# dcmlr/groundgrid

Hardware: NVIDIA H100
Metric: Mpoints/sec segmented (64-beam scan) (higher is better)
Workload: dtype f32/f64

## Files before the change

### groundgrid_b200/csrc/gg_capi.cu

```cuda
#include <cuda.h>
#include <cuda_runtime.h>

#include <cmath>
#include <cstdarg>
#include <cstdio>
#include <algorithm>
#include <atomic>
#include <chrono>
#include <condition_variable>
#include <cstdlib>
#include <cstring>
#include <initializer_list>
#include <mutex>
#include <string>
#include <thread>
#include <utility>
#include <vector>

#include "gg_host.h"
#include "gg_internal.h"

namespace {

thread_local std::string g_last_error;
// ... 1077 lines not shown
    h->have_layer_map = encode_layer_map(h);
    float* expected = nullptr;
    GG_TRY(dev_alloc(h, &expected, N2));
    v.expected = expected;
    GG_TRY(dev_alloc(h, &v.points, S * P));
    GG_TRY(dev_alloc(h, &v.zw, S * P));
    GG_TRY(dev_alloc(h, &v.zsorted, S * P));
    GG_TRY(dev_alloc(h, &v.runj, S * P));
    GG_TRY(dev_alloc(h, &v.rundir, S * P));
    GG_TRY(dev_alloc(h, &v.dist, S * P));
    GG_TRY(dev_alloc(h, &v.code, S * P));
    GG_TRY(dev_alloc(h, &v.labels, S * P));
    GG_TRY(dev_alloc(h, &v.cnt64, S * N2));
    GG_TRY(dev_alloc(h, &v.raw_i, (flags & GG_FLAG_FULL_LAYERS) ? S * N2 : 1));
    GG_TRY(dev_alloc(h, &v.cellstart, S * N2));
    GG_TRY(dev_alloc(h, &v.worklist, S * N2));
    GG_TRY(dev_alloc(h, &v.wl_count, 2 * S));
    v.cell_tiles = (int)((N2 + 4095) / 4096);
    GG_TRY(dev_alloc(h, &v.cell_agg, S * v.cell_tiles * 65));
    GG_TRY(dev_alloc(h, &v.out_index, S * P));
    GG_TRY(dev_alloc(h, &v.out_counts, S * (3 * (size_t)v.out_blocks + 1)));
    GG_TRY(dev_alloc(h, &v.roll_scratch, S * 2 * N2));
    v.out_cloud = nullptr;
    GG_CUDA_TRY(cudaMemset(v.layers, 0, S * v.n_layers * N2 * sizeof(float)));
    GG_CUDA_TRY(cudaMemset(v.cnt64, 0, S * N2 * sizeof(unsigned long long)));
    if (flags & GG_FLAG_FULL_LAYERS) GG_CUDA_TRY(cudaMemset(v.raw_i, 0, S * N2 * sizeof(int)));

    {
        std::vector<float> table;
        gg::build_expected_points(n, table);
        GG_CUDA_TRY(cudaMemcpy(expected, table.data(), N2 * sizeof(float), cudaMemcpyHostToDevice));
        gg::SpiralPlan plan;
        gg::plan_spiral(n, v.k.res_sq, plan);
        GG_TRY(dev_upload(h, &v.level_start, plan.level_start));
        GG_TRY(dev_upload(h, &v.visits, plan.visits, 1));
        v.levels = (int)plan.level_start.size() - 1;
        h->sched_levels = v.levels;
        h->sched_visits = (int)plan.visits.size();
        h->sched_max = plan.max_per_level;
        v.spiral_threads = plan.threads;
        v.spiral_recs = nullptr;
        std::memset(&v.skew, 0, sizeof(v.skew));
        if (plan.kind == gg::SPIRAL_PIPE) {
            const uint32_t* d_rc = nullptr;
            GG_TRY(dev_upload(h, &d_rc, plan.recs, 4));
            v.spiral_recs = reinterpret_cast<const uint4*>(d_rc);
        } else if (plan.kind == gg::SPIRAL_SKEW) {
            const gg::SkewTables& sk = plan.skew;
            gg::SkewView& w = v.skew;
            GG_TRY(dev_upload(h, &w.ph_begin, plan.ph_begin));
            GG_TRY(dev_upload(h, &w.ph_end, plan.ph_end));
            GG_TRY(dev_upload(h, &w.ph_cell0, plan.ph_cell0));
            GG_TRY(dev_upload(h, &w.cell_home, sk.cell_home));
            const uint32_t* d_irr = nullptr;
            GG_TRY(dev_upload(h, &d_irr, plan.irr_blocks, 16));
            float2* d_sk = nullptr;
            float* d_sd = nullptr;
            GG_TRY(dev_alloc(h, &d_sk, S * sk.slots));
            GG_TRY(dev_alloc(h, &d_sd, S * sk.slots));
            GG_CUDA_TRY(cudaMemset(d_sk, 0, S * sk.slots * sizeof(float2)));
            GG_CUDA_TRY(cudaMemset(d_sd, 0, S * sk.slots * sizeof(float)));
            w.sk = d_sk;
            w.sd = d_sd;
            w.slots = sk.slots;
            w.M = plan.M;
            w.phases = plan.phases;
            w.irr_blocks = reinterpret_cast<const uint4*>(d_irr);
            w.irr_max = plan.irr_max;
            w.irr_chunks = plan.irr_chunks;
            w.KP = sk.KP;
            w.rows = sk.rows;
            w.row0 = sk.row0;
            w.lanes = sk.lanes;
            w.levels = sk.levels;
            std::memcpy(w.pattern, sk.pattern, sizeof(sk.pattern));
        }
    }

    if (const char* e = getenv("GG_LAUNCH_UNIT")) h->launch_unit = std::max(1, atoi(e));
    if (const char* e = getenv("GG_HOST_PACK")) {
        h->host_pack = atoi(e) ? 1 : 0;
        h->host_pack_mix = 0;
    }
    v.packed = nullptr;
    if (stream) {
        h->own_streams = false;
        h->n_streams = 1;
        h->streams[0] = static_cast<cudaStream_t>(stream);
    } else {
        int want = 8;
        if (const char* e = getenv("GG_STREAMS")) want = atoi(e);
        h->n_streams = std::max(1, std::min(std::min(want, kStreams), n_slots));
        for (int i = 0; i < h->n_streams; ++i) GG_CUDA_TRY(cudaStreamCreateWithFlags(&h->streams[i], cudaStreamNonBlocking));
    }
    GG_CUDA_TRY(cudaHostAlloc(reinterpret_cast<void**>(&h->h_ring), sizeof(gg::SlotParams) * kRing * S, cudaHostAllocDefault));
    GG_TRY(dev_alloc(h, &h->d_ring, (size_t)kRing * S));
    GG_CUDA_TRY(cudaHostAlloc(reinterpret_cast<void**>(&h->h_dest), sizeof(gg::OutDest) * kRing * S, cudaHostAllocDefault));
    GG_TRY(dev_alloc(h, &h->d_dest, (size_t)kRing * S));
    GG_CUDA_TRY(cudaHostAlloc(reinterpret_cast<void**>(&h->h_unpack), sizeof(gg::UnpackDesc) * kRing * S, cudaHostAllocDefault));
    GG_TRY(dev_alloc(h, &h->d_unpack, (size_t)kRing * S));
    GG_CUDA_TRY(cudaHostAlloc(reinterpret_cast<void**>(&h->h_query), sizeof(gg::QueryDesc) * kRing * S, cudaHostAllocDefault));
    GG_TRY(dev_alloc(h, &h->d_query, (size_t)kRing * S));
    for (int i = 0; i < kRing; ++i) GG_CUDA_TRY(cudaEventCreateWithFlags(&h->ring_ev[i], cudaEventDisableTiming));
    GG_CUDA_TRY(cudaEventCreateWithFlags(&h->caller_in, cudaEventDisableTiming));
    for (int i = 0; i < kStreams; ++i) GG_CUDA_TRY(cudaEventCreateWithFlags(&h->caller_out[i], cudaEventDisableTiming));
    GG_TRY(build_variant(h, 0, h->streams[0]));
// ... 1791 lines not shown
```

### groundgrid_b200/csrc/gg_host.cpp

```cpp
#include <immintrin.h>

#include <algorithm>
#include <cmath>
#include <cstdio>
#include <thread>
#include <cstdint>
#include <cstdlib>
#include <cstring>
#include <vector>

#include <sched.h>

#include "gg_host.h"

namespace gg {

int cells_per_side(double dimension_m, float resolution) {
    return (int)std::round((float)dimension_m / resolution);
}

void build_expected_points(int n, std::vector<float>& table) {
    const float vertical_point_ang_dist = 0.00174532925 * 2;
    table.assign((size_t)n * n, 0.0f);
    const size_t cells = (size_t)n;
// ... 186 lines not shown
    std::vector<Visit> seq;
    seq.reserve(nv);
    std::vector<int> seen((size_t)n * n, 0);
    int max_level = 0;
    auto push = [&](int s, int k, int j, int x, int y) {
        const size_t cell = x + (size_t)y * n;
        const int l = cell_levels[cell][seen[cell]++];
        seq.push_back({s, k, j, x, y, l});
        max_level = std::max(max_level, l);
    };
    for (int k = 0; k < K; ++k) {
        const int p = c - 1 - k, L = 2 * (k + 1), q = p + L;
        for (int j = 0; j < L; ++j) push(0, k, j, p, p + j);
        for (int j = 0; j < L; ++j) push(1, k, j, p + j, p);
        for (int j = 0; j <= L; ++j) push(2, k, j, q, q - j);
        for (int j = 0; j <= L; ++j) push(3, k, j, q - j, q);
    }
    if (seq.size() != nv) return;
    int off[4] = {0, 0, 0, 0};
    const int k_ref = K / 2;
    for (const Visit& v : seq)
        if (v.k == k_ref && v.j == 0) off[v.s] = v.level - 3 * k_ref;
    for (const Visit& v : seq)
        if (v.k >= 4 && v.j == 0 && v.level != 3 * v.k + off[v.s]) return;
    const int LK = 2 * (K + 1);
    t.rows = std::max(max_level, 3 * K + off[3] + LK + 1) + t.row0 + 8;
    t.lanes = 4 * t.KP;
    t.slots = (size_t)4 * t.rows * t.KP;
    auto slot = [&](int s, int k, int level) { return (int)(((size_t)s * t.rows + level + t.row0) * t.KP + (k + 1)); };

    t.cell_home.assign((size_t)n * n * 4, -1);
    auto add_home = [&](int x, int y, int sl) {
        int* h = &t.cell_home[((size_t)x + (size_t)y * n) * 4];
        for (int i = 0; i < 4; ++i)
            if (h[i] < 0) {
                h[i] = sl;
                return;
            }
    };
    for (const Visit& v : seq) add_home(v.x, v.y, slot(v.s, v.k, v.level));
    {
        const int p = 0, k = K, q = p + LK;
        if (q < n) {
            for (int j = 0; j < LK; ++j) add_home(p, p + j, slot(0, k, 3 * k + off[0] + j));
            for (int j = 1; j < LK; ++j) add_home(p + j, p, slot(1, k, 3 * k + off[1] + j));
            for (int j = 0; j <= LK; ++j) add_home(q, q - j, slot(2, k, 3 * k + off[2] + j));
            for (int j = 1; j <= LK; ++j)
                if (!(q - j == p)) add_home(q - j, q, slot(3, k, 3 * k + off[3] + j));
            add_home(p, q, slot(3, k, 3 * k + off[3] + LK));
        }
        for (int s = 0; s < 4; ++s) add_home(c, c, slot(s, -1, -3 + off[s]));
    }
    auto homes = [&](int x, int y) { return &t.cell_home[((size_t)x + (size_t)y * n) * 4]; };

    std::vector<std::vector<std::pair<int, int>>> stat(36);
    auto bump = [&](int idx, int o) {
        for (auto& e : stat[idx])
            if (e.first == o) {
                ++e.second;
                return;
            }
        stat[idx].push_back({o, 1});
    };
    for (const Visit& v : seq) {
        if (v.j < 3 || v.k < 4) continue;
        const int own = slot(v.s, v.k, v.level);
        for (int q = 0; q < 9; ++q) {
            const int* h = homes(v.x - 1 + q % 3, v.y - 1 + q / 3);
            for (int i = 0; i < 4 && h[i] >= 0; ++i) bump(v.s * 9 + q, h[i] - own);
        }
    }
    for (int i = 0; i < 36; ++i) {
        int best = 0, cnt = -1;
        for (auto& e : stat[i])
            if (e.second > cnt) {
                cnt = e.second;
                best = e.first;
            }
        if (cnt < 0) return;
        t.pattern[i] = best;
    }

    std::vector<int> last_level((size_t)n * n, -1000000), last_lane((size_t)n * n, -1);
    t.lane_begin.assign(t.lanes, 0);
    t.lane_end.assign(t.lanes, 0);
    t.lane_cell0.assign(t.lanes, 0);
    std::vector<int> reg_first(t.lanes, -1), reg_last(t.lanes, -1), reg_count(t.lanes, 0);
    struct Irr {
        int level;
        uint32_t w[16];
    };
    std::vector<Irr> irr;
    for (const Visit& v : seq) {
        const int lane = v.s * t.KP + (v.k + 1);
        const int own = slot(v.s, v.k, v.level);
        const size_t cell = v.x + (size_t)v.y * n;
        int nb[9];
        bool regular = true;
        uint32_t rec[4] = {0xffffu, 0xffffu, 0xffffu, 0xffffu};
        int nrec = 0;
        for (int q = 0; q < 9; ++q) {
            const int cx = v.x - 1 + q % 3, cy = v.y - 1 + q / 3;
            const int* h = homes(cx, cy);
            if (h[0] < 0) return;
            const int want = own + t.pattern[v.s * 9 + q];
            bool match = false;
// ... 272 lines not shown
    std::memcpy(dst, t.data(), t.size() * sizeof(float));
    return n;
}

int gg_host_spiral_schedule(int n, int* level_start, int level_cap, uint32_t* visits, int visit_cap, int* n_levels, int* n_visits) {
    std::vector<int> ls;
    std::vector<uint32_t> vs;
    gg::build_spiral_schedule(n, ls, vs);
    *n_levels = (int)ls.size() - 1;
    *n_visits = (int)vs.size();
    if (level_start && level_cap >= (int)ls.size()) std::memcpy(level_start, ls.data(), ls.size() * sizeof(int));
    if (visits && visit_cap >= (int)vs.size()) std::memcpy(visits, vs.data(), vs.size() * sizeof(uint32_t));
    return 0;
}

int gg_host_spiral_records(int n, float resolution, int dist, uint32_t* recs, int rec_cap_words, int* max_recent) {
    std::vector<int> ls;
    std::vector<uint32_t> vs, rc;
    gg::build_spiral_schedule(n, ls, vs);
    int mr = 0;
    const bool ok = gg::build_spiral_records(n, (double)resolution * (double)resolution, ls, vs, dist, rc, mr);
    if (max_recent) *max_recent = mr;
    if (recs && rec_cap_words >= (int)rc.size()) std::memcpy(recs, rc.data(), rc.size() * sizeof(uint32_t));
    return ok ? 1 : 0;
}

int gg_host_spiral_plan(int n, float resolution, int* out) {
    gg::SpiralPlan p;
    gg::plan_spiral(n, (double)resolution * (double)resolution, p);
    const int v[4] = {(int)p.kind, p.threads, p.M, p.phases};
    std::memcpy(out, v, sizeof(v));
    return 0;
}

int gg_host_spiral_skew(int n, int* header, int* pattern, int* lane_begin, int* lane_end, int* cell_home, int* irr_level_start,
                        uint32_t* irr_recs, int irr_cap_words) {
    std::vector<int> ls;
    std::vector<uint32_t> vs;
    gg::build_spiral_schedule(n, ls, vs);
    gg::SkewTables t;
    gg::build_spiral_skew(n, ls, vs, t);
    const int h[10] = {t.ok ? 1 : 0, t.K, t.KP, t.rows, t.levels, t.row0, t.lanes, (int)t.n_irregular, t.max_irr_per_level, (int)t.n_regular};
    std::memcpy(header, h, sizeof(h));
    if (!t.ok) return 0;
    if (pattern) std::memcpy(pattern, t.pattern, sizeof(t.pattern));
    if (lane_begin) std::memcpy(lane_begin, t.lane_begin.data(), t.lane_begin.size() * sizeof(int));
    if (lane_end) std::memcpy(lane_end, t.lane_end.data(), t.lane_end.size() * sizeof(int));
    if (cell_home) std::memcpy(cell_home, t.cell_home.data(), t.cell_home.size() * sizeof(int));
    if (irr_level_start) std::memcpy(irr_level_start, t.irr_level_start.data(), t.irr_level_start.size() * sizeof(int));
    if (irr_recs && irr_cap_words >= (int)t.irr_recs.size()) std::memcpy(irr_recs, t.irr_recs.data(), t.irr_recs.size() * sizeof(uint32_t));
    return 1;
}

int gg_host_decay_confidence(const gg_config* cfg, const float* occ, size_t n, float* out) {
    gg::CfgConst k;
    gg::derive_config(*cfg, k);
    for (size_t i = 0; i < n; ++i) out[i] = gg::decay_confidence(k, occ[i]);
    return 0;
}

int gg_host_skew_visit_confidence(const float* d, const float* occ, size_t n, float* out) {
    for (size_t i = 0; i < n; ++i) out[i] = gg::skew_decays(d[i]) ? d[i] : occ[i];
    return 0;
}

int gg_host_outlier_walk(double dimension_m, float resolution, const double* pos_xy, const float* G, const float* C, double thr, double tol,
                         const float* origin, const float* point, long long from) {
    gg::Const k;
    gg::derive_geometry(dimension_m, resolution, 0, k);
    float vx = point[0] - origin[0], vy = point[1] - origin[1], vz = point[2] - origin[2];
    const float sq = (vx * vx + vy * vy) + vz * vz;
    const float len = std::sqrt(sq);
    vx = vx / len;
    vy = vy / len;
    vz = vz / len;
    if (!(vz < -0.01f)) return -1;
    if (from < 0) return -1;
    const gg::OutlierRay ray{pos_xy[0], pos_xy[1], k.half, k.res, (double)len * (double)len, thr, tol, origin[0], origin[1], origin[2], vx, vy, vz, k.N};
    return gg::outlier_walk(ray, G, C, from > 2147483648LL ? 2147483648u : (unsigned)from) ? 1 : 0;
}

int gg_host_move_map(double res, double* pos_xy, double nx, double ny, int* shift_ij) {
    gg::move_map(res, pos_xy[0], pos_xy[1], nx, ny, shift_ij[0], shift_ij[1]);
    return (shift_ij[0] != 0 || shift_ij[1] != 0) ? 1 : 0;
}

int gg_host_resolve_move(double res, double* pos_xy, double nx, double ny, int* shift_ij) {
    return gg::resolve_move(res, pos_xy[0], pos_xy[1], nx, ny, shift_ij[0], shift_ij[1]);
}

int gg_host_geometry_constants(double dimension_m, float resolution, unsigned flags, double* out) {
    gg::Const k;
    gg::derive_geometry(dimension_m, resolution, flags, k);
    const double v[9] = {(double)k.N, (double)k.N2, (double)k.full_layers, (double)k.res_f, k.res, k.rres, k.len, k.half, k.res_sq};
    std::memcpy(out, v, sizeof(v));
    return 0;
}

int gg_host_config_constants(const gg_config* cfg, double* out) {
    gg::CfgConst k;
    gg::derive_config(*cfg, k);
    const double v[16] = {(double)k.max_ring, (double)k.pc_var_thresh_f, k.min_outlier_conf, k.outlier_tol, k.gp_thresh, k.df_sq, k.mdf_sq,
                          k.mdf10_sq, k.psc_sq, k.occ_factor, k.occ_factor2, k.dec_factor, k.lab_fac, k.lab_thres, k.lab_obs,
                          (double)k.decay_floor_ok};
    std::memcpy(out, v, sizeof(v));
    return 0;
// ... 34 lines not shown
```

### groundgrid_b200/csrc/gg_host.h

```cpp
#pragma once
#include <cstdint>
#include <vector>

#include "gg_internal.h"

namespace gg {
int cells_per_side(double dimension_m, float resolution);
void build_expected_points(int n, std::vector<float>& table);
void derive_geometry(double dimension_m, float resolution, unsigned flags, Const& k);

class ConfigRegistry {
  public:
    void reset(int n_slots, const CfgConst& k);
    int assign(int slot, const CfgConst& k, bool* build);
    void invalidate(int id) { vars_[id].k.reserved = 1; }
    int variant_of(int slot) const { return slot_var_[slot]; }
    const CfgConst& constants(int id) const { return vars_[id].k; }
    int refs(int id) const { return vars_[id].refs; }
    int live() const;
    int ids() const { return (int)vars_.size(); }

  private:
    struct Variant {
        CfgConst k;
        int refs;
    };
    std::vector<Variant> vars_;
    std::vector<int> slot_var_;
};
void move_map(double res, double& px, double& py, double nx, double ny, int& shift_i, int& shift_j);
void build_spiral_schedule(int n, std::vector<int>& level_start, std::vector<uint32_t>& visits);
void pack_cloud_range(const gg_point* src, size_t n, unsigned char* dst, size_t i0, size_t i1);
int usable_cpus();

struct SkewTables {
    bool ok = false;
    int n = 0, K = 0, KP = 0, rows = 0, levels = 0, row0 = 8;
    int lanes = 0;
    size_t slots = 0;
    int pattern[36] = {0};
    int prev_q[4] = {1, 3, 7, 5};
    std::vector<int> lane_begin, lane_end;
    std::vector<int> lane_cell0;
    std::vector<int> cell_home;
    std::vector<int> irr_level_start;
    std::vector<uint32_t> irr_recs;
    int max_irr_per_level = 0;
    size_t n_regular = 0, n_irregular = 0;
};
void build_spiral_skew(int n, const std::vector<int>& level_start, const std::vector<uint32_t>& visits, SkewTables& t);
bool build_spiral_records(int n, double res_sq, const std::vector<int>& level_start, const std::vector<uint32_t>& visits,
                          int dist, std::vector<uint32_t>& recs, int& max_recent);

enum SpiralKind : int { SPIRAL_PLAIN = 0, SPIRAL_PIPE = 1, SPIRAL_SKEW = 2 };
struct SpiralPlan {
    SpiralKind kind = SPIRAL_PLAIN;
    int threads = 0;
    int M = 0, phases = 0;
    std::vector<int> level_start;
    std::vector<uint32_t> visits;
    int max_per_level = 0;
    std::vector<uint32_t> recs;
    SkewTables skew;
    std::vector<int> ph_begin, ph_end, ph_cell0;
    std::vector<uint32_t> irr_blocks;
    int irr_max = 0, irr_chunks = 0;
};
void plan_spiral(int n, double res_sq, SpiralPlan& p);
}

extern "C" {
int gg_host_cells_per_side(double dimension_m, float resolution);
int gg_host_expected_points(double dimension_m, float resolution, float* dst);
int gg_host_spiral_schedule(int n, int* level_start, int level_cap, uint32_t* visits, int visit_cap, int* n_levels, int* n_visits);
int gg_host_spiral_records(int n, float resolution, int dist, uint32_t* recs, int rec_cap_words, int* max_recent);
int gg_host_move_map(double res, double* pos_xy, double nx, double ny, int* shift_ij);
int gg_host_resolve_move(double res, double* pos_xy, double nx, double ny, int* shift_ij);
int gg_host_geometry_constants(double dimension_m, float resolution, unsigned flags, double* out);
int gg_host_config_constants(const gg_config* cfg, double* out);
int gg_host_config_registry(int n_slots, int n_ops, const int* op_slot, const gg_config* op_cfg, int* out);
int gg_host_pack_cloud(const gg_point* src, size_t n, unsigned char* dst);
int gg_host_packer_selftest(int threads, int n_jobs, size_t n_points, int ring_slots, int rounds, int lag);
int gg_host_spiral_plan(int n, float resolution, int* out);
int gg_host_spiral_skew(int n, int* header, int* pattern, int* lane_begin, int* lane_end, int* cell_home, int* irr_level_start, uint32_t* irr_recs, int irr_cap_words);
int gg_host_decay_confidence(const gg_config* cfg, const float* occ, size_t n, float* out);
int gg_host_skew_visit_confidence(const float* d, const float* occ, size_t n, float* out);
int gg_host_outlier_walk(double dimension_m, float resolution, const double* pos_xy, const float* G, const float* C, double thr, double tol,
                         const float* origin, const float* point, long long from);
}
```

### groundgrid_b200/csrc/gg_internal.h

```cpp
#pragma once
#include <cuda.h>
#include <cuda_runtime.h>
#include <stdint.h>

#include <cfloat>

#include "groundgrid_b200.h"

namespace gg {

enum Layer : int {
    L_GROUND = 0,
    L_GROUNDPATCH = 1,
    L_OBSTACLES = 2,
    L_VARIANCE = 3,
    L_MINH = 4,
    L_COUNT = 5,
    L_MAXH = 6,
    L_GCAND = 7,
    L_PLANEDIST = 8,
    L_M2 = 9,
    L_MEAN = 10,
    L_RAW = 11,
    L_NUM = 12,
// ... 25 lines not shown
    double min_outlier_conf, outlier_tol;
    double gp_thresh;
    double df_sq, mdf_sq, mdf10_sq, psc_sq;
    double occ_factor, occ_factor2, dec_factor;
    double lab_fac, lab_thres, lab_obs;
    int decay_floor_ok;
    int reserved;
};
static_assert(sizeof(CfgConst) == 120, "CfgConst has no padding");

struct SlotParams {
    CfgConst cfg;
    const float4* detect_tab;
    double px, py;
    double t20, t21, t22, t23;
    float ox, oy, oz;
    float base_z_f;
    int n_points;
    int shift_i, shift_j;
    int slot;
    const gg_point* src;
    const float* packed;
    int pos;
    int points_layer;
};

struct OutDest {
    uint8_t* labels;
    uint32_t* index;
    gg_point* cloud;
    int* count;
    unsigned select;
    int reserved;
};

constexpr int SPIRAL_THREADS = 512;
constexpr int SPIRAL_PIPE_DIST = 2;
constexpr int SKEW_IRR_THREADS = 64;
constexpr int SKEW_XCH_DEPTH = 2;

struct SkewView {
    float2* sk;
    float* sd;
    size_t slots;
    const int* cell_home;
    const int* ph_begin;
    const int* ph_end;
    const int* ph_cell0;
    int M, phases;
    const uint4* irr_blocks;
    int irr_max, irr_chunks;
    int KP, rows, row0, lanes, levels;
    int pattern[36];
};

struct View {
    Const k;
    float* layers;
    int n_layers;
    const float* expected;
    gg_point* points;
    unsigned char* packed;
    uint2* zw;
    uint32_t* runj;
    float* zsorted;
    uint2* rundir;
    float* dist;
    uint32_t* code;
    uint8_t* labels;
    unsigned long long* cnt64;
    int* raw_i;
    int* cellstart;
    int4* worklist;
    int* wl_count;
    int* cell_agg;
    int cell_tiles;
    uint32_t* out_index;
    int* out_counts;
    gg_point* out_cloud;
    float* roll_scratch;
    size_t pcap;
    int out_blocks;
    const int* level_start;
    const uint32_t* visits;
    int levels;
    const uint4* spiral_recs;
    int spiral_threads;
    SkewView skew;

    __host__ __device__ float* layer(int slot, int l) const { return layers + ((size_t)slot * n_layers + l) * k.N2; }
};

constexpr int RASTER_TILE = 2048;
constexpr int RASTER_THREADS = 256;
constexpr int OUT_TILE = 1024;

enum KernelId : int {
    K_RASTERIZE = 0, K_CELL_TILES, K_CELL_PLACE, K_SCATTER, K_CELL_STATS, K_DETECT, K_SPIRAL, K_LABEL, K_ROLL_GATHER, K_ROLL_COMMIT, K_OUT_COUNT, K_OUT_SCAN,
    K_OUT_WRITE, K_UNPACK, K_TERRAIN, K_EVAL, K_LAYER_COPY, K_LAYER_RANGE, K_LAYER_IMAGE, K_SAMPLE, K_POINT_INFO, K_STAGE_POSES, K_POSE_RESOLVE,
    K_STORE_COUNTS, K_RESET_MAPS, K_STAGE_PARTS, K_STORE_PART_COUNTS, K_STORE_CONFIGS, K_REBUILD_DETECT,
    K_NUM
};

struct Profiler {
    virtual void begin(int kernel_id, cudaStream_t st) = 0;
    virtual void end(int kernel_id, cudaStream_t st) = 0;
    virtual ~Profiler() {}
// ... 266 lines not shown
```

### groundgrid_b200/csrc/gg_kernels.cu

```cuda
#include <cuda.h>

#include <cfloat>
#include <cstddef>
#include <cstdio>

#include "gg_internal.h"

namespace gg {

__device__ __forceinline__ int trunc_index(double v) {
    if (!(v == v)) return 1000000000;
    if (v > 1.0e9) return 1000000000;
    if (v < -1.0e9) return -1000000000;
    return __double2int_rz(v);
}

__device__ __forceinline__ int trunc_quotient(double a, double res, double rres) {
    const double q = __dmul_rn(a, rres);
    const double f = __dsub_rn(q, rint(q));
    if (fabs(q) < 1.0e6 && fabs(f) > 1.0e-6) return __double2int_rz(q);
    return trunc_index(__ddiv_rn(a, res));
}

__device__ __forceinline__ void grid_index(const Const& k, double px, double py, double x, double y, int& ix, int& iy) {
// ... 576 lines not shown
        }
    }
    {
        int rj = 0, pb = 0, pe = cnt;
        if (runs > 1) {
            const uint2 e0 = dir[0];
            pb = (int)(e0.y & RUN_LOW26);
            pe = pb + (int)(e0.y >> 26) + 1;
        }
        float zb[8], zn[8];
        int mb = 0, mnx = 0;
        auto fetch = [&](float* dst, int& m) {
            m = min(8, pe - pb);
#pragma unroll
            for (int q = 0; q < 8; ++q) dst[q] = (q < m) ? zs[pb + q] : 0.0f;
            pb += m;
            if (pb == pe && ++rj < runs) {
                const uint2 en = dir[rj];
                pb = (int)(en.y & RUN_LOW26);
                pe = pb + (int)(en.y >> 26) + 1;
                if (((pb + 8) & ~31) != (pb & ~31)) asm volatile("prefetch.global.L1 [%0];" ::"l"(zs + pb + 8));
            }
        };
        fetch(zb, mb);
        while (mb > 0) {
            fetch(zn, mnx);
#pragma unroll
            for (int q = 0; q < 8; ++q)
                if (q < mb) step(zb[q]);
#pragma unroll
            for (int q = 0; q < 8; ++q) zb[q] = zn[q];
            mb = mnx;
        }
    }
    v.cnt64[coff + cell] = 0ull;
    v.layer(sp.slot, L_COUNT)[cell] = n;
    v.layer(sp.slot, L_VARIANCE)[cell] = __fdiv_rn(m2, __fadd_rn(n, FLT_MIN));
    v.layer(sp.slot, L_MINH)[cell] = mn;
    if (FULL) {
        v.layer(sp.slot, L_M2)[cell] = m2;
        v.layer(sp.slot, L_MEAN)[cell] = mean;
        v.layer(sp.slot, L_GCAND)[cell] = gc;
        v.layer(sp.slot, L_PLANEDIST)[cell] = pdm;
        v.layer(sp.slot, L_MAXH)[cell] = mx;
    }
    }
}

constexpr int DT_X = 32, DT_Y = 8, DT_H = 2;
constexpr int DT_W = DT_X + 2 * DT_H;
constexpr int DT_R = DT_Y + 2 * DT_H;


__device__ __forceinline__ void skew_store_cell(const View& v, const SlotParams& sp, int cell, int x, int y, float g, float c, bool far) {
    const Const& k = v.k;
    const CfgConst& kc = sp.cfg;
    const int4 home = __ldg(reinterpret_cast<const int4*>(v.skew.cell_home) + cell);
    if (home.x < 0) return;
    const int cidx = k.N / 2 - 1;
    if (x == cidx && y == cidx) {
        g = sp.base_z_f;
        c = 1.0f;
    }
    const float d1 = far ? decay_confidence(kc, c) : SKEW_NEAR;
    float2* SK = v.skew.sk + (size_t)sp.slot * v.skew.slots;
    float* SD = v.skew.sd + (size_t)sp.slot * v.skew.slots;
    const float2 gc = make_float2(g, c);
    SK[home.x] = gc;
    SD[home.x] = d1;
    if (home.y >= 0) {
        SK[home.y] = gc;
        SD[home.y] = far ? decay_confidence(kc, d1) : SKEW_NEAR;
    }
    if (home.z >= 0) SK[home.z] = gc;
    if (home.w >= 0) SK[home.w] = gc;
}

constexpr int DTF_S5 = 1, DTF_FAR = 2, DTF_INNER = 4;

__device__ __forceinline__ float4 detect_table_entry(const View& v, const CfgConst& kc, int cell) {
    const Const& k = v.k;
    const int N = k.N;
    const int i = cell % N, j = cell / N;
    const double di = __dsub_rn((double)i, (double)N / 2.0), dj = __dsub_rn((double)j, (double)N / 2.0);
    const float sqdist = (float)__dmul_rn(__dadd_rn(__dmul_rn(di, di), __dmul_rn(dj, dj)), k.res_sq);
    const float e = v.expected[cell];
    int flags = 0;
    if (!((double)sqdist <= kc.psc_sq)) flags |= DTF_S5;
    if (i >= 2 && i < 2 * (N / 2) - 2 && j >= 2 && j < N - 2) flags |= DTF_INNER;
    const int cidx = N / 2 - 1;
    const float fx = __fsub_rn((float)i, (float)cidx), fy = __fsub_rn((float)j, (float)cidx);
    if (__dmul_rn(__dadd_rn(__dmul_rn((double)fx, (double)fx), __dmul_rn((double)fy, (double)fy)), k.res_sq) > 12.0) flags |= DTF_FAR;
    const double S = (flags & DTF_S5) ? 5.0 : 3.0;
    double need = floor(__dmul_rn(__dmul_rn(kc.gp_thresh, S), (double)e));
    need = (need < 3.0) ? 3.0 : need;
    const double a = __dmul_rn((double)sqdist, kc.df_sq);
    const double m = (a < kc.mdf_sq) ? kc.mdf_sq : a;
    const float vt = (float)((kc.mdf10_sq < m) ? kc.mdf10_sq : m);
    return make_float4(__double2float_ru(need), vt, e, __int_as_float(flags));
}

__global__ void k_build_detect_table(View v, const CfgConst kc, float4* __restrict__ tab) {
    const int cell = blockIdx.x * blockDim.x + threadIdx.x;
    if (cell >= v.k.N2) return;
    tab[cell] = detect_table_entry(v, kc, cell);
}

__global__ void __launch_bounds__(256) k_rebuild_detect_tables(View v, const CfgConst* __restrict__ cfgs, const SlotParams* __restrict__ batch) {
    const SlotParams& p = batch[blockIdx.y];
    if (!p.n_points) return;
    const int cell = blockIdx.x * 256 + threadIdx.x;
    if (cell >= v.k.N2) return;
    const_cast<float4*>(p.detect_tab)[cell] = detect_table_entry(v, cfgs[p.slot], cell);
}

template <int S>
__device__ __forceinline__ bool detect_patch(const CfgConst& kc, const float (*sP)[DT_W], const float (*sPV)[DT_W], const float (*sPM)[DT_W],
                                             const float (*sM)[DT_W], int li, int lj, float variance, float need, float vt, float e, float& g,
                                             float& c) {
    constexpr int H = S / 2;
    const int r0 = li - H, c0 = lj - H;
    const float psum = TreeSum<0, S * S>::run([&](int q) { return sP[c0 + q / S][r0 + q % S]; });
    const float oc = c, og = g;

    if (psum < need) return false;

    float localmin = sM[c0][r0];
#pragma unroll
// ... 46 lines not shown
    const int gi = i0 - DT_H + tx, gj = j0 - DT_H + ty;
    const bool col0 = gi >= 0 && gi < N, col1 = tx < 2 * DT_H && gi + DT_X < N;
    const bool row0 = gj >= 0 && gj < N, row1 = ty < 2 * DT_H && gj + DT_Y < N;
    const int o = gi + gj * N;
    const bool in[4] = {col0 && row0, col1 && row0, col0 && row1, col1 && row1};
    const int off[4] = {o, o + DT_X, o + DT_Y * N, o + DT_Y * N + DT_X};
    float tp[4], tv[4], tm[4];
#pragma unroll
    for (int u = 0; u < 4; ++u) {
        tp[u] = in[u] ? P[off[u]] : 0.0f;
        tv[u] = in[u] ? V[off[u]] : 0.0f;
        tm[u] = in[u] ? M[off[u]] : FLT_MAX;
        if (recompute) tv[u] = __fdiv_rn(tv[u], __fadd_rn(tp[u], FLT_MIN));
    }
    const int i = i0 + tx, j = j0 + ty;
    const bool live = i < N && j < N;
    const int cell = i + j * N;
    float g = 0.0f, c = 0.0f, variance = 0.0f;
    float4 tb = make_float4(0.0f, 0.0f, 0.0f, 0.0f);
    if (live) {
        g = L0[L_GROUND * N2 + cell];
        c = L0[L_GROUNDPATCH * N2 + cell];
        variance = V[cell];
        tb = __ldg(sp.detect_tab + cell);
        if (recompute) {
            variance = __fdiv_rn(variance, __fadd_rn(P[cell], FLT_MIN));
            L0[L_VARIANCE * N2 + cell] = variance;
        }
    }
#pragma unroll
    for (int u = 0; u < 4; ++u) {
        const bool mine = ((u & 1) == 0 || tx < 2 * DT_H) && ((u & 2) == 0 || ty < 2 * DT_H);
        if (mine) {
            const int li = (u & 1) ? DT_X + tx : tx, lj = (u & 2) ? ty + DT_Y : ty;
            sP[lj][li] = tp[u];
            sPV[lj][li] = __fmul_rn(tp[u], tv[u]);
            sPM[lj][li] = __fmul_rn(tp[u], tm[u]);
            sM[lj][li] = tm[u];
        }
    }
    __syncthreads();
    if (!live) return;
    const int flags = __float_as_int(tb.w);
    if (flags & DTF_INNER) {
        const int li = threadIdx.x + DT_H, lj = threadIdx.y + DT_H;
        const bool changed = (flags & DTF_S5) ? detect_patch<5>(kc, sP, sPV, sPM, sM, li, lj, variance, tb.x, tb.y, tb.z, g, c)
                                              : detect_patch<3>(kc, sP, sPV, sPM, sM, li, lj, variance, tb.x, tb.y, tb.z, g, c);
        if (changed) {
            L0[L_GROUND * N2 + cell] = g;
            L0[L_GROUNDPATCH * N2 + cell] = c;
        }
    }
    if (v.skew.sk) {
        skew_store_cell(v, sp, cell, i, j, g, c, (flags & DTF_FAR) != 0);
    } else if (v.spiral_recs) {
        const float d1 = decay_confidence(kc, c);
        float* D1 = v.roll_scratch + (size_t)sp.slot * 2 * k.N2;
        D1[cell] = d1;
        if (i == j) D1[k.N2 + cell] = decay_confidence(kc, d1);
    }
}

__device__ __forceinline__ uint32_t smem_u32(const void* p) { return (uint32_t)__cvta_generic_to_shared(p); }

__device__ __forceinline__ void mbar_init(uint64_t* bar, int count) {
    asm volatile("mbarrier.init.shared::cta.b64 [%0], %1;" ::"r"(smem_u32(bar)), "r"(count));
    asm volatile("fence.mbarrier_init.release.cluster;" ::: "memory");
}
__device__ __forceinline__ void mbar_expect_tx(uint64_t* bar, uint32_t bytes) {
    asm volatile("mbarrier.arrive.expect_tx.shared::cta.b64 _, [%0], %1;" ::"r"(smem_u32(bar)), "r"(bytes) : "memory");
}
__device__ __forceinline__ void mbar_wait(uint64_t* bar, uint32_t parity) {
    asm volatile(
        "{\n"
        ".reg .pred p;\n"
        "WAIT_LOOP:\n"
        "mbarrier.try_wait.parity.shared::cta.b64 p, [%0], %1;\n"
        "@p bra WAIT_DONE;\n"
        "bra WAIT_LOOP;\n"
        "WAIT_DONE:\n"
        "}\n" ::"r"(smem_u32(bar)),
        "r"(parity)
        : "memory");
}
__device__ __forceinline__ void tma_load_3d(void* dst, const CUtensorMap* map, uint64_t* bar, int c0, int c1, int c2) {
    asm volatile("cp.async.bulk.tensor.3d.shared::cluster.global.tile.mbarrier::complete_tx::bytes [%0], [%1, {%3, %4, %5}], [%2];" ::"r"(smem_u32(dst)),
                 "l"(map), "r"(smem_u32(bar)), "r"(c0), "r"(c1), "r"(c2)
                 : "memory");
}

constexpr int DT_HX = 4;
constexpr int DT_WT = DT_X + 2 * DT_HX;
constexpr int DT_WC = DT_WT - 4;
constexpr int DT_WB = DT_WT - 2;

struct __align__(128) DetectRaw {
    float P[DT_R][DT_WT];
    float V[DT_R][DT_WT];
    float M[DT_R][DT_WT];
};
struct __align__(128) DetectTile {
    DetectRaw raw[2];
    float C3[DT_R][DT_WT], C5[DT_R][DT_WT];
    float N3[DT_R][DT_WT], N5[DT_R][DT_WT];
    float QV[DT_R][DT_WT], PV2[DT_R][DT_WT], TV[DT_R][DT_WT];
    float QM[DT_R][DT_WT], PM2[DT_R][DT_WT], TM[DT_R][DT_WT];
};
// ... 9 lines not shown
    const float s18_7 = __fadd_rn(__fadd_rn(QQ(3, 3), __fadd_rn(QQ(4, 3), QQ(0, 4))), __fadd_rn(PP(1, 4), PP(3, 4)));
    return __fadd_rn(__fadd_rn(s0_6, s6_6), __fadd_rn(s12_6, s18_7));
#undef TT
}
__device__ __forceinline__ float tree9s(const float (*Q)[DT_WT], const float (*P2)[DT_WT], int r0, int c0) {
    const float s0_4 = __fadd_rn(PP(0, 0), __fadd_rn(QQ(2, 0), QQ(0, 1)));
    const float s4_5 = __fadd_rn(PP(1, 1), __fadd_rn(QQ(0, 2), PP(1, 2)));
    return __fadd_rn(s0_4, s4_5);
#undef QQ
#undef PP
}

template <int S>
__device__ __forceinline__ bool detect_decide(const CfgConst& kc, float psum, float localmin, float sumPV, float sumPM, float centerP, float variance, float vt,
                                              float e, float& g, float& c) {
    const float oc = c, og = g;
    const float maxVar = (centerP >= kc.pc_var_thresh_f) ? variance : __fdiv_rn(sumPV, psum);
    const float groundlevel = __fdiv_rn(sumPM, psum);
    const float gd = __fmul_rn(__fsub_rn(groundlevel, og), __fmul_rn(2.0f, oc));
    const float groundDiff = (gd < 1.0f) ? 1.0f : gd;
    if ((double)oc > 0.5 && (double)groundlevel >= __dadd_rn((double)og, kc.outlier_tol)) return false;
    if ((double)vt > __dmul_rn((double)maxVar, (double)maxVar) && maxVar > 0.0f &&
        (double)psum > __dmul_rn((double)__fmul_rn(__fmul_rn(groundDiff, e), (float)S), kc.gp_thresh)) {
        float nc = 1.0f;
        if (!(kc.occ_factor > 0.0 && (double)psum >= kc.occ_factor)) {
            const double ncd = __ddiv_rn((double)psum, kc.occ_factor);
            nc = (float)((1.0 < ncd) ? 1.0 : ncd);
        }
        const float num = __fadd_rn(__fmul_rn(groundlevel, nc), __fmul_rn(__fmul_rn(oc, og), 2.0f));
        const float den = __fadd_rn(nc, __fmul_rn(oc, 2.0f));
        g = __fdiv_rn(num, den);
        const double cd = __dmul_rn(__dadd_rn(__ddiv_rn((double)psum, kc.occ_factor2), (double)oc), 0.5);
        c = (float)((1.0 < cd) ? 1.0 : cd);
        return true;
    }
    if (localmin < og) {
        g = localmin;
        const float t = __fadd_rn(oc, 0.1f);
        c = (0.5f < t) ? 0.5f : t;
        return true;
    }
    return false;
}

constexpr int DT_TILES = 4;
constexpr float DT_EXACT_COUNT = 524288.0f;

__device__ __forceinline__ float min_skip_nan(float a, float b) { return (b < a || a != a) ? b : a; }

__global__ void __launch_bounds__(DT_X* DT_Y, 5) k_detect_tma(View v, const SlotParams* __restrict__ batch, const __grid_constant__ CUtensorMap tmap,
                                                             int count_layer, bool recompute) {
    __shared__ DetectTile s;
    __shared__ __align__(8) uint64_t s_bar[2];
    const SlotParams& sp = batch[blockIdx.z];
    const Const& k = v.k;
    const CfgConst& kc = sp.cfg;
    const int N = k.N, N2 = k.N2;
    const int i0 = blockIdx.x * DT_X;
    const int tx = threadIdx.x, ty = threadIdx.y, tid = ty * DT_X + tx;
    const int tile0 = blockIdx.y * DT_TILES;
    const int n_tiles = min(DT_TILES, (N + DT_Y - 1) / DT_Y - tile0);
    const int plane0 = sp.slot * v.n_layers;
    auto issue = [&](int kk) {
        constexpr uint32_t kBytes = 3u * DT_R * DT_WT * sizeof(float);
        DetectRaw& r = s.raw[kk & 1];
        uint64_t* bar = &s_bar[kk & 1];
        const int j0 = (tile0 + kk) * DT_Y;
        mbar_expect_tx(bar, kBytes);
        tma_load_3d(&r.P[0][0], &tmap, bar, i0 - DT_HX, j0 - DT_H, plane0 + count_layer);
        tma_load_3d(&r.V[0][0], &tmap, bar, i0 - DT_HX, j0 - DT_H, plane0 + (recompute ? L_M2 : L_VARIANCE));
        tma_load_3d(&r.M[0][0], &tmap, bar, i0 - DT_HX, j0 - DT_H, plane0 + L_MINH);
    };
    if (tid == 0) {
        mbar_init(&s_bar[0], 1);
        mbar_init(&s_bar[1], 1);
    }
    __syncthreads();
    if (tid == 0) issue(0);
    float* const L0 = v.layer(sp.slot, 0);
    const int i = i0 + tx;
    const int li = tx + DT_HX, lj = ty + DT_H;
    for (int kk = 0; kk < n_tiles; ++kk) {
        if (tid == 0 && kk + 1 < n_tiles) issue(kk + 1);
        const DetectRaw& raw = s.raw[kk & 1];
        const int j = (tile0 + kk) * DT_Y + ty;
        const bool live = i < N && j < N;
        const int cell = i + j * N;
        float g = 0.0f, c = 0.0f;
        float4 tb = make_float4(0.0f, 0.0f, 0.0f, 0.0f);
        if (live) {
            g = L0[L_GROUND * N2 + cell];
            c = L0[L_GROUNDPATCH * N2 + cell];
            tb = __ldg(sp.detect_tab + cell);
        }
        const int flags = __float_as_int(tb.w);
        mbar_wait(&s_bar[kk & 1], (uint32_t)((kk >> 1) & 1));
        if (recompute) {
            DetectRaw& rw = s.raw[kk & 1];
            for (int p = tid; p < DT_R * DT_WT; p += DT_X * DT_Y) {
                const int row = p / DT_WT, col = p % DT_WT;
                rw.V[row][col] = __fdiv_rn(rw.V[row][col], __fadd_rn(rw.P[row][col], FLT_MIN));
            }
            asm volatile("fence.proxy.async.shared::cta;" ::: "memory");
            __syncthreads();
            if (live) L0[L_VARIANCE * N2 + cell] = rw.V[lj][li];
        }

        bool exact = true;
        for (int p = tid; p < DT_R * DT_WC; p += DT_X * DT_Y) {
            const int row = p / DT_WC, col = p % DT_WC;
            float a[5];
#pragma unroll
            for (int q = 0; q < 5; ++q) {
                a[q] = raw.P[row][col + q];
                exact = exact && a[q] >= 0.0f && a[q] <= DT_EXACT_COUNT && a[q] == truncf(a[q]);
            }
            const float c3 = __fadd_rn(__fadd_rn(a[0], a[1]), a[2]);
            s.C3[row][col] = c3;
            s.C5[row][col] = __fadd_rn(__fadd_rn(c3, a[3]), a[4]);
        }
        exact = __syncthreads_and(exact);
        const bool inner = live && (flags & DTF_INNER);
        const bool s5 = (flags & DTF_S5) != 0;
        float psum = 0.0f;
        if (inner && !exact) {
            if (s5)
                psum = TreeSum<0, 25>::run([&](int q) { return raw.P[lj - 2 + q / 5][li - 2 + q % 5]; });
            else
                psum = TreeSum<0, 9>::run([&](int q) { return raw.P[lj - 1 + q / 3][li - 1 + q % 3]; });
        } else if (inner) {
            if (s5) {
                const int r0 = li - 2, c0 = lj - 2;
                psum = __fadd_rn(__fadd_rn(__fadd_rn(s.C5[c0][r0], s.C5[c0 + 1][r0]), __fadd_rn(s.C5[c0 + 2][r0], s.C5[c0 + 3][r0])), s.C5[c0 + 4][r0]);
            } else {
                const int r0 = li - 1, c0 = lj - 1;
                psum = __fadd_rn(__fadd_rn(s.C3[c0][r0], s.C3[c0 + 1][r0]), s.C3[c0 + 2][r0]);
            }
        }
        const bool cand = inner && !(psum < tb.x);
        const bool any = __syncthreads_or(cand);
        bool changed = false;
        if (any) {
            for (int p = tid; p < DT_R * DT_WB; p += DT_X * DT_Y) {
                const int row = p / DT_WB, col = p % DT_WB;
                float qv[3], qm[3], m[5];
#pragma unroll
                for (int q = 0; q < 5; ++q) m[q] = raw.M[row][col + q];
#pragma unroll
                for (int q = 0; q < 3; ++q) {
                    const float pp = raw.P[row][col + q];
                    const float vv = raw.V[row][col + q];
                    qv[q] = __fmul_rn(pp, vv);
                    qm[q] = __fmul_rn(pp, m[q]);
                }
                s.QV[row][col] = qv[0];
                s.QM[row][col] = qm[0];
                const float pv12 = __fadd_rn(qv[1], qv[2]), pm12 = __fadd_rn(qm[1], qm[2]);
                s.PV2[row][col] = __fadd_rn(qv[0], qv[1]);
                s.PM2[row][col] = __fadd_rn(qm[0], qm[1]);
                s.TV[row][col] = __fadd_rn(qv[0], pv12);
                s.TM[row][col] = __fadd_rn(qm[0], pm12);
                const float n3 = min_skip_nan(min_skip_nan(m[0], m[1]), m[2]);
                s.N3[row][col] = n3;
                s.N5[row][col] = min_skip_nan(min_skip_nan(n3, m[3]), m[4]);
            }
            __syncthreads();
            if (cand) {
                const float variance = raw.V[lj][li], centerP = raw.P[lj][li];
                if (s5) {
                    const int r0 = li - 2, c0 = lj - 2;
                    float localmin = s.N5[c0][r0];
#pragma unroll
                    for (int q = 1; q < 5; ++q) {
                        const float t = s.N5[c0 + q][r0];
                        localmin = (t < localmin) ? t : localmin;
                    }
                    const float m0 = raw.M[c0][r0];
                    localmin = (m0 != m0) ? m0 : localmin;
                    changed = detect_decide<5>(kc, psum, localmin, tree25(s.QV, s.PV2, s.TV, r0, c0), tree25(s.QM, s.PM2, s.TM, r0, c0), centerP, variance,
                                               tb.y, tb.z, g, c);
                } else {
                    const int r0 = li - 1, c0 = lj - 1;
                    float localmin = s.N3[c0][r0];
#pragma unroll
                    for (int q = 1; q < 3; ++q) {
                        const float t = s.N3[c0 + q][r0];
                        localmin = (t < localmin) ? t : localmin;
                    }
                    const float m0 = raw.M[c0][r0];
                    localmin = (m0 != m0) ? m0 : localmin;
                    changed = detect_decide<3>(kc, psum, localmin, tree9s(s.QV, s.PV2, r0, c0), tree9s(s.QM, s.PM2, r0, c0), centerP, variance, tb.y, tb.z, g, c);
                }
            }
        }
        if (live) {
            if (changed) {
                L0[L_GROUND * N2 + cell] = g;
                L0[L_GROUNDPATCH * N2 + cell] = c;
            }
            if (v.skew.sk) {
                skew_store_cell(v, sp, cell, i, j, g, c, (flags & DTF_FAR) != 0);
            } else if (v.spiral_recs) {
                const float d1 = decay_confidence(kc, c);
                float* D1 = v.roll_scratch + (size_t)sp.slot * 2 * k.N2;
                D1[cell] = d1;
                if (i == j) D1[k.N2 + cell] = decay_confidence(kc, d1);
            }
        }
        __syncthreads();
    }
}

int launch_build_detect_table(const View& v, const CfgConst& c, float4* tab, cudaStream_t st) {
    k_build_detect_table<<<(v.k.N2 + 255) / 256, 256, 0, st>>>(v, c, tab);
    return 1;
}

__global__ void __launch_bounds__(SPIRAL_THREADS) k_spiral(View v, const SlotParams* __restrict__ batch) {
    const SlotParams& sp = batch[blockIdx.x];
    const Const& k = v.k;
    const CfgConst& kc = sp.cfg;
    const int N = k.N;
    float* G = v.layer(sp.slot, L_GROUND);
    float* C = v.layer(sp.slot, L_GROUNDPATCH);
    const int cidx = N / 2 - 1;
    if (threadIdx.x == 0) {
        C[cidx + cidx * N] = 1.0f;
        G[cidx + cidx * N] = sp.base_z_f;
    }
    __syncthreads();
    const float fc = (float)cidx;
    for (int lvl = 0; lvl < v.levels; ++lvl) {
        const int b = v.level_start[lvl], e = v.level_start[lvl + 1];
        for (int t = b + threadIdx.x; t < e; t += SPIRAL_THREADS) {
            const uint32_t vis = v.visits[t];
            const int x = (int)(vis & 0xffffu), y = (int)(vis >> 16);
            float cc[9], pr[9];
#pragma unroll
            for (int q = 0; q < 9; ++q) {
                const int g = (x - 1 + q % 3) + (y - 1 + q / 3) * N;
                cc[q] = C[g];
                pr[q] = __fmul_rn(cc[q], G[g]);
            }
            const float h = G[x + y * N];
            const float occ = cc[4];
            const float s = __fadd_rn(tree9(cc), FLT_MIN);
            const float avg = __fdiv_rn(tree9(pr), s);
            G[x + y * N] = __fadd_rn(__fmul_rn(__fsub_rn(1.0f, occ), avg), __fmul_rn(occ, h));
            const float fx = __fsub_rn((float)x, fc), fy = __fsub_rn((float)y, fc);
            const double d2 = __dmul_rn(__dadd_rn(__dmul_rn((double)fx, (double)fx), __dmul_rn((double)fy, (double)fy)), k.res_sq);
            if (d2 > 12.0) {
                const double o = (double)occ;
                const double dec = __dsub_rn(o, __ddiv_rn(o, kc.dec_factor));
                C[x + y * N] = (float)((dec < 0.001) ? 0.001 : dec);
            }
        }
        __syncthreads();
    }
}

// ... 1417 lines not shown
```

Measured before the change: 4969.

## Compute regular skew homes analytically and coalesce skew-slot stores via shared staging

Adds an analytic formula for each cell's primary skew home slot and uses a per-cell bitmask so that only irregular cells read the 16-byte cell_home table. The tiled detect kernel stages each cell's (g, c, decay, slot) in shared memory, then permutes which thread writes which entry so that writes to skew slots along ring sides fall on more contiguous addresses. The aim is to cut global gather loads and scattered stores in the detect pass. In exchange it adds a shared-memory staging buffer, an extra barrier per tile, more integer arithmetic per cell, and an asm barrier on tid.

```diff
diff --git a/groundgrid_b200/csrc/gg_capi.cu b/groundgrid_b200/csrc/gg_capi.cu
--- a/groundgrid_b200/csrc/gg_capi.cu
+++ b/groundgrid_b200/csrc/gg_capi.cu
@@ -1153,6 +1153,10 @@
             GG_TRY(dev_upload(h, &w.ph_end, plan.ph_end));
             GG_TRY(dev_upload(h, &w.ph_cell0, plan.ph_cell0));
             GG_TRY(dev_upload(h, &w.cell_home, sk.cell_home));
+            GG_TRY(dev_upload(h, &w.home_irr, sk.home_irr));
+            w.home_words = sk.home_words;
+            w.K = sk.K;
+            std::memcpy(w.off, sk.off, sizeof(sk.off));
             const uint32_t* d_irr = nullptr;
             GG_TRY(dev_upload(h, &d_irr, plan.irr_blocks, 16));
             float2* d_sk = nullptr;
diff --git a/groundgrid_b200/csrc/gg_host.cpp b/groundgrid_b200/csrc/gg_host.cpp
--- a/groundgrid_b200/csrc/gg_host.cpp
+++ b/groundgrid_b200/csrc/gg_host.cpp
@@ -262,6 +262,15 @@
         for (int s = 0; s < 4; ++s) add_home(c, c, slot(s, -1, -3 + off[s]));
     }
     auto homes = [&](int x, int y) { return &t.cell_home[((size_t)x + (size_t)y * n) * 4]; };
+    std::memcpy(t.off, off, sizeof(off));
+    t.home_words = (n + 31) / 32;
+    t.home_irr.assign((size_t)n * t.home_words, 0u);
+    for (int y = 0; y < n; ++y)
+        for (int x = 0; x < n; ++x) {
+            const int* h = homes(x, y);
+            if (h[0] != skew_regular_home(n, K, t.KP, t.rows, t.row0, t.off, x, y) || h[1] >= 0)
+                t.home_irr[(size_t)y * t.home_words + x / 32] |= 1u << (x % 32);
+        }
 
     std::vector<std::vector<std::pair<int, int>>> stat(36);
     auto bump = [&](int idx, int o) {
@@ -640,6 +649,38 @@
     return 1;
 }
 
+int gg_host_skew_homes(int n, int* homes, int* n_table) {
+    std::vector<int> ls;
+    std::vector<uint32_t> vs;
+    gg::build_spiral_schedule(n, ls, vs);
+    gg::SkewTables t;
+    gg::build_spiral_skew(n, ls, vs, t);
+    if (!t.ok) return 0;
+    gg::SkewView w;
+    std::memset(&w, 0, sizeof(w));
+    w.cell_home = t.cell_home.data();
+    w.home_irr = t.home_irr.data();
+    w.home_words = t.home_words;
+    w.K = t.K;
+    w.KP = t.KP;
+    w.rows = t.rows;
+    w.row0 = t.row0;
+    std::memcpy(w.off, t.off, sizeof(t.off));
+    int table = 0;
+    for (int y = 0; y < n; ++y)
+        for (int x = 0; x < n; ++x) {
+            const int4 h = gg::skew_home(w, n, x, y);
+            int* o = homes + ((size_t)x + (size_t)y * n) * 4;
+            o[0] = h.x;
+            o[1] = h.y;
+            o[2] = h.z;
+            o[3] = h.w;
+            table += (t.home_irr[(size_t)y * t.home_words + x / 32] >> (x % 32)) & 1u;
+        }
+    *n_table = table;
+    return 1;
+}
+
 int gg_host_decay_confidence(const gg_config* cfg, const float* occ, size_t n, float* out) {
     gg::CfgConst k;
     gg::derive_config(*cfg, k);
diff --git a/groundgrid_b200/csrc/gg_host.h b/groundgrid_b200/csrc/gg_host.h
--- a/groundgrid_b200/csrc/gg_host.h
+++ b/groundgrid_b200/csrc/gg_host.h
@@ -43,6 +43,9 @@
     std::vector<int> lane_begin, lane_end;
     std::vector<int> lane_cell0;
     std::vector<int> cell_home;
+    int off[4] = {0, 0, 0, 0};
+    int home_words = 0;
+    std::vector<uint32_t> home_irr;
     std::vector<int> irr_level_start;
     std::vector<uint32_t> irr_recs;
     int max_irr_per_level = 0;
@@ -83,6 +86,7 @@
 int gg_host_packer_selftest(int threads, int n_jobs, size_t n_points, int ring_slots, int rounds, int lag);
 int gg_host_spiral_plan(int n, float resolution, int* out);
 int gg_host_spiral_skew(int n, int* header, int* pattern, int* lane_begin, int* lane_end, int* cell_home, int* irr_level_start, uint32_t* irr_recs, int irr_cap_words);
+int gg_host_skew_homes(int n, int* homes, int* n_table);
 int gg_host_decay_confidence(const gg_config* cfg, const float* occ, size_t n, float* out);
 int gg_host_skew_visit_confidence(const float* d, const float* occ, size_t n, float* out);
 int gg_host_outlier_walk(double dimension_m, float resolution, const double* pos_xy, const float* G, const float* C, double thr, double tol,
diff --git a/groundgrid_b200/csrc/gg_internal.h b/groundgrid_b200/csrc/gg_internal.h
--- a/groundgrid_b200/csrc/gg_internal.h
+++ b/groundgrid_b200/csrc/gg_internal.h
@@ -101,7 +101,46 @@
     int irr_max, irr_chunks;
     int KP, rows, row0, lanes, levels;
     int pattern[36];
-};
+    const uint32_t* home_irr;
+    int home_words;
+    int K;
+    int off[4];
+};
+
+__host__ __device__ __forceinline__ int skew_regular_home(int n, int K, int KP, int rows, int row0, const int* off, int x, int y) {
+    const int c = n / 2 - 1;
+    const int ax = x > c ? x - c : c - x, ay = y > c ? y - c : c - y;
+    const int k = (ax > ay ? ax : ay) - 1;
+    if (k < 0 || k > K) return -1;
+    const int p = c - 1 - k, q = c + 1 + k;
+    int s, j;
+    if (x == p && y < q) {
+        s = 0;
+        j = y - p;
+    } else if (y == p && x < q) {
+        s = 1;
+        j = x - p;
+    } else if (x == q) {
+        s = 2;
+        j = q - y;
+    } else {
+        s = 3;
+        j = q - x;
+    }
+    return (s * rows + 3 * k + off[s] + j + row0) * KP + k + 1;
+}
+
+__host__ __device__ __forceinline__ int4 skew_home(const SkewView& w, int n, int x, int y) {
+    if ((w.home_irr[y * w.home_words + (x >> 5)] >> (x & 31)) & 1u) {
+#ifdef __CUDA_ARCH__
+        return __ldg(reinterpret_cast<const int4*>(w.cell_home) + x + y * n);
+#else
+        const int* h = w.cell_home + 4 * ((size_t)x + (size_t)y * n);
+        return make_int4(h[0], h[1], h[2], h[3]);
+#endif
+    }
+    return make_int4(skew_regular_home(n, w.K, w.KP, w.rows, w.row0, w.off, x, y), -1, -1, -1);
+}
 
 struct View {
     Const k;
diff --git a/groundgrid_b200/csrc/gg_kernels.cu b/groundgrid_b200/csrc/gg_kernels.cu
--- a/groundgrid_b200/csrc/gg_kernels.cu
+++ b/groundgrid_b200/csrc/gg_kernels.cu
@@ -652,10 +652,9 @@
 constexpr int DT_R = DT_Y + 2 * DT_H;
 
 
-__device__ __forceinline__ void skew_store_cell(const View& v, const SlotParams& sp, int cell, int x, int y, float g, float c, bool far) {
+__device__ __forceinline__ void skew_store_homes(const View& v, const SlotParams& sp, int4 home, int x, int y, float g, float c, bool far) {
     const Const& k = v.k;
     const CfgConst& kc = sp.cfg;
-    const int4 home = __ldg(reinterpret_cast<const int4*>(v.skew.cell_home) + cell);
     if (home.x < 0) return;
     const int cidx = k.N / 2 - 1;
     if (x == cidx && y == cidx) {
@@ -674,6 +673,56 @@
     }
     if (home.z >= 0) SK[home.z] = gc;
     if (home.w >= 0) SK[home.w] = gc;
+}
+__device__ __forceinline__ void skew_store_cell(const View& v, const SlotParams& sp, int x, int y, float g, float c, bool far) {
+    skew_store_homes(v, sp, skew_home(v.skew, v.k.N, x, y), x, y, g, c, far);
+}
+
+__device__ __forceinline__ void skew_store_tile(const View& v, const SlotParams& sp, float4* stage, bool live, int x, int y, float g, float c,
+                                                bool far) {
+    const int N = v.k.N;
+    const int cidx = N / 2 - 1;
+    int slot = -1;
+    float d = SKEW_NEAR;
+    if (live) {
+        const int4 home = skew_home(v.skew, N, x, y);
+        if (home.x >= 0) {
+            if (x == cidx && y == cidx) {
+                g = sp.base_z_f;
+                c = 1.0f;
+            }
+            if (far) d = decay_confidence(sp.cfg, c);
+            slot = home.x;
+            if (home.y >= 0) {
+                float2* SK = v.skew.sk + (size_t)sp.slot * v.skew.slots;
+                const float2 gc = make_float2(g, c);
+                SK[home.y] = gc;
+                v.skew.sd[(size_t)sp.slot * v.skew.slots + home.y] = far ? decay_confidence(sp.cfg, d) : SKEW_NEAR;
+                if (home.z >= 0) SK[home.z] = gc;
+                if (home.w >= 0) SK[home.w] = gc;
+            }
+        }
+    }
+    const int tx = threadIdx.x, ty = threadIdx.y;
+    const int ax = abs(x - tx + DT_X / 2 - cidx), ay = abs(y - ty + DT_Y / 2 - cidx);
+    const int lane = tx, w = ty;
+    int lx, ly;
+    if (ay > ax) {
+        ly = lane & 7;
+        lx = (w * 4 + (lane >> 3) + 4 * ly) & (DT_X - 1);
+    } else {
+        const int h = lane & 1;
+        ly = (w >> 1) + 4 * h;
+        lx = ((w & 1) * 16 + (lane >> 1) + h) & (DT_X - 1);
+    }
+    stage[ty * DT_X + tx] = make_float4(g, c, d, __int_as_float(slot));
+    __syncthreads();
+    const float4 e = stage[ly * DT_X + lx];
+    const int sl = __float_as_int(e.w);
+    if (sl >= 0) {
+        v.skew.sk[(size_t)sp.slot * v.skew.slots + sl] = make_float2(e.x, e.y);
+        v.skew.sd[(size_t)sp.slot * v.skew.slots + sl] = e.z;
+    }
 }
 
 constexpr int DTF_S5 = 1, DTF_FAR = 2, DTF_INNER = 4;
@@ -826,7 +875,7 @@
         }
     }
     if (v.skew.sk) {
-        skew_store_cell(v, sp, cell, i, j, g, c, (flags & DTF_FAR) != 0);
+        skew_store_cell(v, sp, i, j, g, c, (flags & DTF_FAR) != 0);
     } else if (v.spiral_recs) {
         const float d1 = decay_confidence(kc, c);
         float* D1 = v.roll_scratch + (size_t)sp.slot * 2 * k.N2;
@@ -942,6 +991,7 @@
                                                              int count_layer, bool recompute) {
     __shared__ DetectTile s;
     __shared__ __align__(8) uint64_t s_bar[2];
+    __shared__ float4 s_stage[DT_X * DT_Y];
     const SlotParams& sp = batch[blockIdx.z];
     const Const& k = v.k;
     const CfgConst& kc = sp.cfg;
@@ -973,6 +1023,8 @@
     for (int kk = 0; kk < n_tiles; ++kk) {
         if (tid == 0 && kk + 1 < n_tiles) issue(kk + 1);
         const DetectRaw& raw = s.raw[kk & 1];
+        int tile_tid = tid;
+        asm volatile("" : "+r"(tile_tid));
         const int j = (tile0 + kk) * DT_Y + ty;
         const bool live = i < N && j < N;
         const int cell = i + j * N;
@@ -987,7 +1039,7 @@
         mbar_wait(&s_bar[kk & 1], (uint32_t)((kk >> 1) & 1));
         if (recompute) {
             DetectRaw& rw = s.raw[kk & 1];
-            for (int p = tid; p < DT_R * DT_WT; p += DT_X * DT_Y) {
+            for (int p = tile_tid; p < DT_R * DT_WT; p += DT_X * DT_Y) {
                 const int row = p / DT_WT, col = p % DT_WT;
                 rw.V[row][col] = __fdiv_rn(rw.V[row][col], __fadd_rn(rw.P[row][col], FLT_MIN));
             }
@@ -997,7 +1049,7 @@
         }
 
         bool exact = true;
-        for (int p = tid; p < DT_R * DT_WC; p += DT_X * DT_Y) {
+        for (int p = tile_tid; p < DT_R * DT_WC; p += DT_X * DT_Y) {
             const int row = p / DT_WC, col = p % DT_WC;
             float a[5];
 #pragma unroll
@@ -1031,7 +1083,7 @@
         const bool any = __syncthreads_or(cand);
         bool changed = false;
         if (any) {
-            for (int p = tid; p < DT_R * DT_WB; p += DT_X * DT_Y) {
+            for (int p = tile_tid; p < DT_R * DT_WB; p += DT_X * DT_Y) {
                 const int row = p / DT_WB, col = p % DT_WB;
                 float qv[3], qm[3], m[5];
 #pragma unroll
@@ -1083,19 +1135,17 @@
                 }
             }
         }
-        if (live) {
-            if (changed) {
-                L0[L_GROUND * N2 + cell] = g;
-                L0[L_GROUNDPATCH * N2 + cell] = c;
-            }
-            if (v.skew.sk) {
-                skew_store_cell(v, sp, cell, i, j, g, c, (flags & DTF_FAR) != 0);
-            } else if (v.spiral_recs) {
-                const float d1 = decay_confidence(kc, c);
-                float* D1 = v.roll_scratch + (size_t)sp.slot * 2 * k.N2;
-                D1[cell] = d1;
-                if (i == j) D1[k.N2 + cell] = decay_confidence(kc, d1);
-            }
+        if (live && changed) {
+            L0[L_GROUND * N2 + cell] = g;
+            L0[L_GROUNDPATCH * N2 + cell] = c;
+        }
+        if (v.skew.sk) {
+            skew_store_tile(v, sp, s_stage, live, i, j, g, c, (flags & DTF_FAR) != 0);
+        } else if (live && v.spiral_recs) {
+            const float d1 = decay_confidence(kc, c);
+            float* D1 = v.roll_scratch + (size_t)sp.slot * 2 * k.N2;
+            D1[cell] = d1;
+            if (i == j) D1[k.N2 + cell] = decay_confidence(kc, d1);
         }
         __syncthreads();
     }
```

Result: faster. 5255, median of 6 (+5.8%).
